# TorontoDeepLearning/convnet

Hardware: AMD Instinct MI355X
Metric: images/sec (fprop+bprop+wgrad) AlexNet 224x224 bs=256 (higher is better)
Workload: dtype f32

## Files before the change

convnet_amd/csrc/elementwise.hip:

```cpp
#include <cfloat>
#include <climits>
#include <cmath>

#include "common.h"

namespace chip {

using f32x4 = __attribute__((ext_vector_type(4))) float;

constexpr int kThreads = 256;
constexpr int kMaxBlocks = 2048;

inline int blocks_for(size_t work_items) {
  size_t b = (work_items + kThreads - 1) / kThreads;
  if (b > kMaxBlocks) b = kMaxBlocks;
  if (b < 1) b = 1;
  return (int)b;
}

template <typename F>
__global__ void map2_kernel(float* __restrict__ out, const float* a, const float* b, size_t n, bool vec, F f) {
  const size_t tid = (size_t)blockIdx.x * blockDim.x + threadIdx.x, stride = (size_t)gridDim.x * blockDim.x;
  if (vec) {
    const size_t n4 = n >> 2;
// ... 194 lines not shown
}

__global__ void add_row_kernel(float* __restrict__ out, const float* __restrict__ mat, const float* __restrict__ vec, int rows,
                               size_t n, float mult, bool vec4) {
  const size_t tid = (size_t)blockIdx.x * blockDim.x + threadIdx.x, stride = (size_t)gridDim.x * blockDim.x;
  if (vec4) {
    for (size_t i = tid; i < (n >> 2); i += stride) {
      const float b = mult * vec[(i << 2) / rows];
      f32x4 v = reinterpret_cast<const f32x4*>(mat)[i];
      v = v + b;
      reinterpret_cast<f32x4*>(out)[i] = v;
    }
  } else {
    for (size_t i = tid; i < n; i += stride) out[i] = mat[i] + mult * vec[i / rows];
  }
}

int add_row(cudamat* mat, cudamat* vec, cudamat* target, float mult) {
  if (!mat->on_device || !vec->on_device || !target->on_device) return ERROR_NOT_ON_DEVICE;
  if (mat->is_trans) return ERROR_TRANSPOSED;
  if (mat->size[1] != vec->size[1] || vec->size[0] != 1 || mat->size[0] != target->size[0] || mat->size[1] != target->size[1])
    return ERROR_INCOMPATIBLE_DIMENSIONS;
  const size_t n = numel(mat);
  const bool v4 = (mat->size[0] & 3) == 0 && aligned16(mat->data_device) && aligned16(target->data_device);
  hipLaunchKernelGGL(add_row_kernel, dim3(blocks_for(n / 4 + 1)), dim3(kThreads), 0, stream(), target->data_device, mat->data_device,
                     vec->data_device, mat->size[0], n, mult, v4);
  return launch_status();
}

__device__ __forceinline__ void sgd_one(float& g, float& w, float& h, float l2, float clip, float eps, float mom);

template <bool DO_SGD>
__global__ void rows_sq_kernel(float* __restrict__ g, float* __restrict__ w, float* __restrict__ h, int rows, int cols, int chunk,
                               float* __restrict__ partial, float l2, float clip, float eps, float mom) {
  const int r = blockIdx.x * blockDim.x + threadIdx.x;
  if (r >= rows) return;
  const int c0 = blockIdx.y * chunk, c1 = min(cols, c0 + chunk);
  float s = 0.f;
  for (int c = c0; c < c1; ++c) {
    const size_t i = (size_t)r + (size_t)rows * c;
    float wv = w[i];
    if (DO_SGD) {
      float gv = g[i], hv = h[i];
      sgd_one(gv, wv, hv, l2, clip, eps, mom);
      g[i] = gv;
      h[i] = hv;
      w[i] = wv;
    }
    s += wv * wv;
  }
  partial[(size_t)blockIdx.y * rows + r] = s;
}

template <bool DO_SGD>
__global__ void rows_sq4_kernel(float* __restrict__ g, float* __restrict__ w, float* __restrict__ h, int rows, int cols, int chunk,
                                float* __restrict__ partial, float l2, float clip, float eps, float mom) {
  const int r = 4 * (blockIdx.x * blockDim.x + threadIdx.x);
  if (r >= rows) return;
  const int c0 = blockIdx.y * chunk, c1 = min(cols, c0 + chunk);
  f32x4 s = {0.f, 0.f, 0.f, 0.f};
  auto one = [&](int c) {
    const size_t i = (size_t)r + (size_t)rows * c;
    f32x4 wv = *reinterpret_cast<f32x4*>(w + i);
    if (DO_SGD) {
      f32x4 gv = *reinterpret_cast<f32x4*>(g + i), hv = *reinterpret_cast<f32x4*>(h + i);
#pragma unroll
      for (int e = 0; e < 4; ++e) {
        float a = gv[e], b = wv[e], d = hv[e];
        sgd_one(a, b, d, l2, clip, eps, mom);
        gv[e] = a; wv[e] = b; hv[e] = d;
      }
      *reinterpret_cast<f32x4*>(g + i) = gv;
      *reinterpret_cast<f32x4*>(h + i) = hv;
      *reinterpret_cast<f32x4*>(w + i) = wv;
    }
    s += wv * wv;
  };
  int c = c0;
  for (; c + 1 < c1; c += 2) {
    one(c);
    one(c + 1);
  }
  if (c < c1) one(c);
  *reinterpret_cast<f32x4*>(partial + (size_t)blockIdx.y * rows + r) = s;
}

__global__ void row_factor_kernel(const float* __restrict__ partial, int nchunks, int rows, float norm, int constraint, float* __restrict__ factor) {
  __shared__ float sh[4][64];
  const int r = blockIdx.x * 64 + (threadIdx.x & 63), q = threadIdx.x >> 6;
  float s = 0.f;
  if (r < rows)
    for (int k = q; k < nchunks; k += 4) s += partial[(size_t)k * rows + r];
  sh[q][threadIdx.x & 63] = s;
  __syncthreads();
  if (q != 0 || r >= rows) return;
  s = sqrtf((sh[0][threadIdx.x] + sh[1][threadIdx.x]) + (sh[2][threadIdx.x] + sh[3][threadIdx.x]));
  factor[r] = (constraint == 1 || s > norm) ? norm / s : 1.f;
}

__global__ void row_scale_kernel(const float* __restrict__ src, float* __restrict__ dst, int rows, int cols, int chunk, const float* __restrict__ factor) {
  const int r = blockIdx.x * blockDim.x + threadIdx.x;
  const float f = r < rows ? factor[r] : 1.f;
  const bool in_place = src == dst;
  if (in_place && !__syncthreads_or(f != 1.f)) return;
  if (r >= rows) return;
  const int c0 = blockIdx.y * chunk, c1 = min(cols, c0 + chunk);
  for (int c = c0; c < c1; ++c) {
    const size_t i = (size_t)r + (size_t)rows * c;
    dst[i] = src[i] * f;
  }
}

inline int rows_normlimit(float* g, float* w_in, float* w_out, float* h, int rows, int cols, float norm, int constraint, bool do_sgd,
                          float l2, float clip, float eps, float mom) {
  int chunk = 64;
  while ((long)divup(rows, 256) * divup(cols, chunk) > 4096 && chunk < cols) chunk *= 2;
  const int nchunks = divup(cols, chunk);
  float* partial = static_cast<float*>(workspace(sizeof(float) * ((size_t)nchunks * rows + rows)));
  float* factor = partial + (size_t)nchunks * rows;
  dim3 grid(divup(rows, 256), nchunks);
  const bool v4 = (rows & 3) == 0 && aligned16(w_in) && (!do_sgd || (aligned16(g) && aligned16(h)));
  KernelTimer timer(do_sgd ? "rows_sq_kernel<sgd> + row_scale_kernel" : "rows_sq_kernel + row_scale_kernel", do_sgd ? "sgd_normlimit" : "normlimit", 0.0,
                    4.0 * (double)rows * cols * (do_sgd ? 7 : 3));
  if (v4) {
    const dim3 g4(divup(rows / 4, 64), nchunks);
    if (do_sgd)
      hipLaunchKernelGGL(rows_sq4_kernel<true>, g4, dim3(64), 0, stream(), g, w_in, h, rows, cols, chunk, partial, l2, clip, eps, mom);
    else
      hipLaunchKernelGGL(rows_sq4_kernel<false>, g4, dim3(64), 0, stream(), nullptr, w_in, nullptr, rows, cols, chunk, partial, 0.f, 0.f, 0.f, 0.f);
  } else if (do_sgd)
    hipLaunchKernelGGL(rows_sq_kernel<true>, grid, dim3(256), 0, stream(), g, w_in, h, rows, cols, chunk, partial, l2, clip, eps, mom);
  else
    hipLaunchKernelGGL(rows_sq_kernel<false>, grid, dim3(256), 0, stream(), nullptr, w_in, nullptr, rows, cols, chunk, partial, 0.f, 0.f, 0.f, 0.f);
  hipLaunchKernelGGL(row_factor_kernel, dim3(divup(rows, 64)), dim3(256), 0, stream(), partial, nchunks, rows, norm, constraint, factor);
  hipLaunchKernelGGL(row_scale_kernel, grid, dim3(256), 0, stream(), w_in, w_out, rows, cols, chunk, factor);
  return launch_status();
}

__global__ void normlimit_cols_kernel(const float* __restrict__ mat, float* __restrict__ target, int rows, float norm, int constraint) {
  __shared__ float sh[8];
  const float* col = mat + (size_t)blockIdx.x * rows;
  float* out = target + (size_t)blockIdx.x * rows;
  float s = 0.f;
  for (int i = threadIdx.x; i < rows; i += blockDim.x) s += col[i] * col[i];
  s = sqrtf(block_sum(s, sh));
  const float sc = (constraint == 1 || s > norm) ? norm / s : 1.f;
  for (int i = threadIdx.x; i < rows; i += blockDim.x) out[i] = col[i] * sc;
}

struct SoftmaxOut {
  float* probs;
  float* deriv;
  float* correct;
};

template <int G>
__global__ void __launch_bounds__(G * 32) softmax_rows_kernel(const float* logits, const float* __restrict__ labels, SoftmaxOut o, int rows, int cols, float deriv_scale) {
  __shared__ float red[G][33];
  __shared__ int redi[G][33];
  const int r = threadIdx.x & 31, g = threadIdx.x >> 5;
  const int row = blockIdx.x * 32 + r;
  const bool ok = row < rows;
  float mx = -FLT_MAX;
  int am = 0x7fffffff;
  if (ok)
    for (int j = g; j < cols; j += G) {
      const float v = logits[(size_t)j * rows + row];
      if (v > mx) { mx = v; am = j; }
    }
  red[g][r] = mx;
  redi[g][r] = am;
  __syncthreads();
  mx = red[0][r];
  am = redi[0][r];
#pragma unroll
  for (int k = 1; k < G; ++k) {
    const float v = red[k][r];
    const int a = redi[k][r];
    if (v > mx || (v == mx && a < am)) { mx = v; am = a; }
  }
  __syncthreads();
  float s = 0.f;
// ... 872 lines not shown
```

convnet_amd/csrc/gather_gemm.h:

```cpp
#pragma once
#include <cmath>
#include <cstring>
#include <type_traits>

#include "common.h"

namespace chip {

using f32x16 = __attribute__((ext_vector_type(16))) float;
using u32x4 = __attribute__((ext_vector_type(4))) unsigned;
using f32x4 = __attribute__((ext_vector_type(4))) float;

constexpr int BK = 16;

#ifdef CONVNET_GG_TRACE
constexpr bool kTrace = CONVNET_GG_TRACE >= 2;
__device__ unsigned long long* g_gg_trace = nullptr;
#else
constexpr bool kTrace = false;
#endif
__device__ __forceinline__ unsigned long long trace_clock() {
#ifdef CONVNET_GG_TRACE
  return __builtin_amdgcn_s_memtime();
#else
// ... 338 lines not shown

template <typename Acc>
__device__ __forceinline__ Acc split_mac(const Split8& a, const Split8& b, Acc v) {
  v = mma_bf16(a.m, b.m, v);
  v = mma_bf16(a.h, b.l, v);
  v = mma_bf16(a.l, b.h, v);
  v = mma_bf16(a.h, b.m, v);
  v = mma_bf16(a.m, b.h, v);
  v = mma_bf16(a.h, b.h, v);
  return v;
}

struct GGTile {
  const float* A;
  int K, GX, G, TX, TYX, y0, x0, dy0, dx0, ncols, col_tiles;
  int L, tsplit;
};
__device__ __forceinline__ bool gg_select_tile(const GGParams& p, const GGClassTable& ct, GGTile& t) {
  t.A = p.A; t.K = p.K; t.GX = p.GX; t.G = p.G; t.TX = p.TX; t.TYX = p.TYX; t.y0 = p.y0; t.x0 = p.x0; t.dy0 = p.dy0; t.dx0 = p.dx0;
  t.ncols = p.ncols; t.col_tiles = p.col_tiles; t.tsplit = -1;
  if (ct.n > 0) {
    const int b = blockIdx.x;
    if (b >= ct.c[ct.n - 1].tile_end) return false;
    int c = 0;
    while (b >= ct.c[c].tile_end) ++c;
    const int cbeg = c > 0 ? ct.c[c - 1].tile_end : 0;
    {
      const int i = b - cbeg, T = ct.c[c].tile_end - cbeg;
      const int q = T >> 3, m = T & 7, r = i & 7;
      t.L = r * q + (r < m ? r : m) + (i >> 3);
    }
    const GGClass& k = ct.c[c];
    t.A = k.A; t.K = k.K; t.GX = k.GX; t.G = k.G; t.TX = k.TX; t.TYX = k.TYX;
    t.y0 = k.y0; t.x0 = k.x0; t.dy0 = k.dy0; t.dx0 = k.dx0; t.ncols = k.ncols; t.col_tiles = k.col_tiles;
  } else if (p.tail_splits > 1) {
    const int k = blockIdx.x & 7, i = blockIdx.x >> 3;
    if (i < p.tail_tf8) {
      t.L = k * p.tail_tf8 + i;
    } else {
      const int j = k * p.tail_tt8 + (i - p.tail_tf8);
      if (j >= (p.row_tiles * t.col_tiles - p.tail_first) * p.tail_splits) return false;
      t.L = p.tail_first + j / p.tail_splits;
      t.tsplit = j % p.tail_splits;
    }
  } else {
    const int tiles = p.row_tiles * t.col_tiles;
    const int per = (tiles + 7) >> 3;
    t.L = xcd_remap(blockIdx.x, tiles);
    if (t.L >= tiles || (int)blockIdx.x >= per * 8) return false;
  }
  return true;
}

constexpr int kTailFixParts = 4;
template <int WR, int WC, int MT, int CW, bool VEC>
__global__ __launch_bounds__(WR* WC * 64) void gg_tail_fix_kernel(const GGParams p) {
  constexpr int NT = WR * WC * 64, NTC = CW / 32, ROWS = WR * MT * 32;
  using fvec = __attribute__((ext_vector_type(NTC))) float;
  const int tile = blockIdx.x / kTailFixParts, part = blockIdx.x % kTailFixParts;
  const int L = p.tail_first + tile;
  const int tid = threadIdx.x;
  const int reg_lo = part * (16 / kTailFixParts), reg_hi = reg_lo + 16 / kTailFixParts;
  f32x16 acc[MT][NTC];
  const float* pp = p.tail_partial + (size_t)tile * p.tail_splits * (size_t)(ROWS * WC * CW);
#pragma unroll
  for (int t = 0; t < MT; ++t)
#pragma unroll
    for (int reg = 0; reg < 16; ++reg) {
      if (reg < reg_lo || reg >= reg_hi) continue;
      fvec v = *reinterpret_cast<const fvec*>(pp + ((size_t)(t * 16 + reg) * NT + tid) * NTC);
      for (int sp = 1; sp < p.tail_splits; ++sp)
        v += *reinterpret_cast<const fvec*>(pp + (size_t)sp * (ROWS * WC * CW) + ((size_t)(t * 16 + reg) * NT + tid) * NTC);
#pragma unroll
      for (int u = 0; u < NTC; ++u) acc[t][u][reg] = v[u];
    }
  gg_epilogue<WR, WC, MT, CW, VEC>(p, acc, L % p.row_tiles, L / p.row_tiles, 0, p.ncols, p.GX, p.G, p.dy0, p.dx0, reg_lo, reg_hi);
}

struct PatchBank {
  const float* W;
  int F, C, Ky, Kx, cy, cx, sy, sx, TYc, TXc;
  bool dgrad;
};
void filter_planes_rt_launch(const PatchBank& bank, void* out, int TYX, int TH, const char* op);
void filter_planes_gk_launch(const float* W, void* out, int F, int K, int KP, int TH, const char* op);
bool patch_shape_ok(GGParams& p, size_t dst_elems);
void patch_run(GGParams& p, size_t dst_elems, const char* op, double flops, const PatchBank& bank);
bool patch_classes_ok(const GGParams& base, const GGClassTable& ct);
void patch_run_classes(GGParams& p, GGClassTable& ct, const char* op, double flops, double exec);

bool gfc_try(const float* images, const float* filters, const float* bias, float* targets, int N, int C, int H, int W, int F, int Ky, int Kx,
             int sy, int sx, int pady, int padx, int My, int Mx, float scaleTargets, int relu, double flops);

struct WGParams {
  const float* src;
  const float* dout;
  float* dst;
  float* partial;
  const float* zero;
  float* bias_dst;
  int K, F, N;
  int GX, M;
  int TX, TYX;
  int SH, SW;
  int ssy, ssx, y0, x0;
  int nchunk;
  int chunks_total;
  int chunks_per_split;
  int splits;
  int k_tiles, f_tiles;
  float scaleTargets, scaleOutput;
  int prio;
  int wide;
};

constexpr int WG_NB = 32;
constexpr int WG_PITCH = WG_NB + 4;

void wg_reduce_launch(const WGParams& p, size_t total, int splits, int groups, const char* op);
float* wg_batch_partial(const WGParams& p, size_t total, int splits);
bool wgw_try(WGParams& p, bool vec, bool split_products, const char* op, double flops, double exec);

void gg_reduce_launch(const GGParams& p, size_t dst_elems, int splits, const char* op);

inline double gg_split_time(int tiles, int sp, double slots, double tile_flops, double block_rate, size_t dst_elems) {
  const double rounds = std::ceil(tiles * (double)sp / slots);
  double t = rounds * (tile_flops / sp) / block_rate;
  if (sp > 1) t += sizeof(float) * (double)dst_elems * (2.0 * sp + 1) / 4.0e12 + 4e-6;
  return t;
// ... 44 lines not shown
```

convnet_amd/csrc/gather_gemm.hip:

```cpp
#include <algorithm>
#include <array>
#include <cmath>
#include <map>
#include <vector>
#include <cstdlib>
#include <string>
#include <type_traits>

#include "common.h"

#include "gather_gemm.h"

namespace chip {

template <int WR, int WC, int MT, int CW, bool A_KCONTIG, bool VEC, bool O3 = false, bool SPLIT = false>
__global__ __launch_bounds__(WR* WC * 64, (O3 ? 3 : 2)) void gg_kernel(const GGParams pin, const GGClassTable ct) {
  constexpr int NT = WR * WC * 64;
  constexpr int NTC = CW / 32, CW4 = CW / 4;
  using fvec = __attribute__((ext_vector_type(NTC))) float;
  constexpr int ROWS = WR * MT * 32;
  constexpr int APITCH = A_KCONTIG ? (BK + 4) : ROWS;
  constexpr int A_STAGE = A_KCONTIG ? ROWS * APITCH : BK * ROWS;
  constexpr int B_STAGE = WC * BK * CW;
  constexpr int NA = ((A_KCONTIG ? ROWS * (BK / 4) : BK * (ROWS / 4)) + NT - 1) / NT;
// ... 733 lines not shown
#pragma unroll
    for (int t = 0; t < MT; ++t) a[0][t] = ar[lh * ROWS + t * 32];
    b4[0] = *reinterpret_cast<const fvec*>(bs + lh * BROW);
    static_for<0, BK / 2>([&](auto KK) __attribute__((always_inline)) {
      constexpr int kk = decltype(KK)::value;
      constexpr int cur = kk & 1, nxt = cur ^ 1;
      if constexpr (kk + 1 < BK / 2) {
        const int krow = 2 * (kk + 1) + lh;
#pragma unroll
        for (int t = 0; t < MT; ++t) a[nxt][t] = ar[krow * ROWS + t * 32];
        b4[nxt] = *reinterpret_cast<const fvec*>(bs + krow * BROW);
      }
      __builtin_amdgcn_sched_barrier(0);
#pragma unroll
      for (int t = 0; t < MT; ++t)
#pragma unroll
        for (int u = 0; u < NTC; ++u)
          acc[t][u] = __builtin_amdgcn_mfma_f32_32x32x2f32(a[cur][t], b4[cur][u], acc[t][u], 0, 0, 0);
    });
    stage = stage == ST - 1 ? 0 : stage + 1;
    __syncthreads();
  }

  if (tsplit >= 0) {
    float* pp = p.tail_partial + ((size_t)(L - p.tail_first) * p.tail_splits + tsplit) * (size_t)(ROWS * WC * CW);
#pragma unroll
    for (int t = 0; t < MT; ++t)
#pragma unroll
      for (int reg = 0; reg < 16; ++reg) {
        fvec v;
#pragma unroll
        for (int u = 0; u < NTC; ++u) v[u] = acc[t][u][reg];
        *reinterpret_cast<fvec*>(pp + ((size_t)(t * 16 + reg) * NC + tid) * NTC) = v;
      }
    return;
  }
  gg_epilogue<WR, WC, MT, CW, true>(p, acc, row_tile, col_tile, split, T.ncols, T.GX, T.G, T.dy0, T.dx0);
}

__global__ void gg_reduce_kernel(float* __restrict__ dst, const float* __restrict__ partial, const float* __restrict__ bias,
                                 size_t total, size_t slab, int splits, size_t per_row, float scaleTargets, int relu,
                                 const float* __restrict__ mask, float post_scale) {
  for (size_t i = (size_t)blockIdx.x * blockDim.x + threadIdx.x; i < total; i += (size_t)gridDim.x * blockDim.x) {
    float s = 0.f;
    for (int k = 0; k < splits; ++k) s += partial[(size_t)k * slab + i];
    if (scaleTargets != 0.f) s = scaleTargets * dst[i] + s;
    if (bias) s += bias[i / per_row];
    if (relu) s = s > 0.f ? s : 0.f;
    if (mask) s = mask[i] > 0.f ? s * post_scale : 0.f;
    dst[i] = s;
  }
}

__global__ void dgrad_filter_kernel(const float* __restrict__ W, float* __restrict__ Wt, int F, int C, int Ky, int Kx, int cy,
                                    int cx, int sy, int sx, int TYc, int TXc, int tap_major) {
  const size_t total = (size_t)C * TXc * TYc * F;
  for (size_t i = (size_t)blockIdx.x * blockDim.x + threadIdx.x; i < total; i += (size_t)gridDim.x * blockDim.x) {
    const int c = i % C;
    size_t r = i / C;
    int a, b, f;
    if (tap_major) {
      const int f16 = r % 16;
      r /= 16;
      const int tap = r % (TXc * TYc);
      const int fb = r / (TXc * TYc);
      f = fb * 16 + f16;
      a = tap / TXc;
      b = tap - a * TXc;
    } else {
      b = r % TXc;
      r /= TXc;
      a = r % TYc;
      f = r / TYc;
    }
    Wt[i] = W[(size_t)f + (size_t)F * ((cx + sx * b) + Kx * ((cy + sy * a) + Ky * c))];
  }
}

__global__ void filter_tapmajor_kernel(const float* __restrict__ W, float* __restrict__ Wt, int F, int C, int TYX) {
  const size_t total = (size_t)F * C * TYX;
  for (size_t i = (size_t)blockIdx.x * blockDim.x + threadIdx.x; i < total; i += (size_t)gridDim.x * blockDim.x) {
    const int f = i % F;
    size_t r = i / F;
    const int c16 = r % 16;
    r /= 16;
    const int tap = r % TYX;
    const int c = (int)(r / TYX) * 16 + c16;
    Wt[i] = W[(size_t)f + (size_t)F * (tap + (size_t)TYX * c)];
  }
}

template <int WM, int WN, int MT, int NTL, bool VEC, int TS, bool SPLIT = false>
__global__ __launch_bounds__(WM* WN * 64) void wg_kernel(const WGParams p) {
  constexpr int NT = WM * WN * 64;
  constexpr int KT = WM * MT * TS;
  constexpr int FT = WN * NTL * TS;
  constexpr int LH = 64 / TS;
  using facc = __attribute__((ext_vector_type(TS == 32 ? 16 : 4))) float;
  constexpr int PITCH = VEC ? WG_NB : WG_PITCH;
  constexpr int A_STAGE = KT * PITCH, B_STAGE = FT * PITCH;
  constexpr int NA = (KT * 8 + NT - 1) / NT, NB = (FT * 8 + NT - 1) / NT;
  extern __shared__ __attribute__((aligned(16))) float smem[];
  float* As = smem;
  float* Bs = smem + 2 * A_STAGE;

  const int tiles = p.k_tiles * p.f_tiles;
// ... 250 lines not shown
        if (fin) {
          v = v * p.scaleOutput;
          if (p.scaleTargets != 0.f) v = p.scaleTargets * ld4(dp) + v;
        }
        st4(dp, v);
      }
      return;
    }
  }
#pragma unroll
  for (int u = 0; u < NTL; ++u) {
    const int f = f0 + (wn * NTL + u) * TS + li;
    if (f >= p.F) continue;
#pragma unroll
    for (int t = 0; t < MT; ++t) {
#pragma unroll
      for (int reg = 0; reg < (TS == 32 ? 16 : 4); ++reg) {
        const int k = kc0 + (wm * MT + t) * TS + (TS == 32 ? (reg & 3) + 8 * (reg >> 2) + 4 * lh : 4 * lh + reg);
        if (k >= KB) continue;
        float* dp = (fin && k == p.K) ? p.bias_dst + f : out + (size_t)k * p.F + f;
        float v = acc[t][u][reg];
        if (fin) {
          v *= p.scaleOutput;
          if (p.scaleTargets != 0.f) v = p.scaleTargets * (*dp) + v;
        }
        *dp = v;
      }
    }
  }
}

__global__ void wg_reduce_group_kernel(float* __restrict__ stage, const float* __restrict__ partial, size_t total, int splits, int per) {
  const int g = blockIdx.y;
  const int k0 = g * per, k1 = min(splits, k0 + per);
  for (size_t i = (size_t)blockIdx.x * blockDim.x + threadIdx.x; i < total; i += (size_t)gridDim.x * blockDim.x) {
    float s = 0.f;
    for (int k = k0; k < k1; ++k) s += partial[(size_t)k * total + i];
    stage[(size_t)g * total + i] = s;
  }
}

__global__ void wg_reduce_kernel(float* __restrict__ dst, float* __restrict__ dst2, const float* __restrict__ partial, size_t total,
                                 size_t main, int splits, float scaleTargets, float scaleOutput) {
  for (size_t i = (size_t)blockIdx.x * blockDim.x + threadIdx.x; i < total; i += (size_t)gridDim.x * blockDim.x) {
    float s = 0.f;
    for (int k = 0; k < splits; ++k) s += partial[(size_t)k * total + i];
    s *= scaleOutput;
    float* d = i < main ? dst + i : dst2 + (i - main);
    if (scaleTargets != 0.f) s = scaleTargets * (*d) + s;
    *d = s;
  }
}

__global__ void __launch_bounds__(256) dot_generic_kernel(const float* __restrict__ a, const float* __restrict__ b, float* __restrict__ c, int m, int n,
                                                          int k, int ld1, int ld2, int t1, int t2, float beta, float alpha) {
  __shared__ float As[32][33], Bs[32][33];
  const int tx = threadIdx.x & 31, ty = threadIdx.x >> 5;
  const int i0 = blockIdx.x * 32, j0 = blockIdx.y * 32;
  float acc[4] = {0.f, 0.f, 0.f, 0.f};
  for (int l0 = 0; l0 < k; l0 += 32) {
    for (int r = ty; r < 32; r += 8) {
      if (t1) {
        const int i = i0 + r, l = l0 + tx;
        As[tx][r] = (i < m && l < k) ? a[(size_t)l + (size_t)ld1 * i] : 0.f;
      } else {
        const int i = i0 + tx, l = l0 + r;
        As[r][tx] = (i < m && l < k) ? a[(size_t)i + (size_t)ld1 * l] : 0.f;
      }
      if (t2) {
        const int j = j0 + tx, l = l0 + r;
        Bs[r][tx] = (j < n && l < k) ? b[(size_t)j + (size_t)ld2 * l] : 0.f;
      } else {
        const int j = j0 + r, l = l0 + tx;
        Bs[tx][r] = (j < n && l < k) ? b[(size_t)l + (size_t)ld2 * j] : 0.f;
      }
    }
    __syncthreads();
#pragma unroll 8
    for (int l = 0; l < 32; ++l) {
      const float av = As[l][tx];
#pragma unroll
      for (int q = 0; q < 4; ++q) acc[q] = fmaf(av, Bs[l][ty + 8 * q], acc[q]);
    }
    __syncthreads();
  }
  const int i = i0 + tx;
  if (i < m) {
#pragma unroll
    for (int q = 0; q < 4; ++q) {
      const int j = j0 + ty + 8 * q;
      if (j < n) {
        float* d = c + (size_t)i + (size_t)m * j;
        *d = (beta != 0.f ? beta * (*d) : 0.f) + alpha * acc[q];
      }
    }
  }
}

namespace {

constexpr int kTargetBlocks = 512;

struct GGTimer {
  const char* op;
  double flops, exec;
};
// ... 155 lines not shown
  const int tiles = p.row_tiles * p.col_tiles;
  const int kchunks = divup(p.K, BK);
  const bool no_o3 = CHIP_DIAG_KNOB("CONVNET_GG_NO_O3", 0) != 0;
  const bool o3 = !no_o3 && !gg_split_mode() && vec && !AK && WR == 2 && WC == 2 && MT == 2 && CW == 128 && tiles >= 2 * 768 && p.KC == 0;
  int slots = o3 ? 768 : kTargetBlocks;
  if constexpr (kHasProducer<WC, CW, AK>) {
    if (p.KC > 0) slots = ggp_slots<WR, WC, MT, CW>(gg_split_mode(), p.apre != 0);
  }
  const double block_rate = gg_split_mode() ? 190e12 / slots : 64.0 * 4 * 2.2e9 * 0.8 / 2;
  const double flops = 2.0 * ROWS * (WC * (double)CW) * (double)p.K;
  const bool may_tail = dst_elems > 0 && gg_partial_last_round(tiles, slots, kchunks) && !CHIP_DIAG_KNOB("CONVNET_GG_NO_TAIL_SPLIT", 0);
  double best_t = 1e30;
  int splits = gg_split_k(tiles, slots, flops, block_rate, dst_elems, kchunks, kchunks, &best_t);
  int tail_s_instead = 0;
  if (splits > 1 && may_tail) {
    const int full = (tiles / slots) * slots, rem = tiles - full;
    const double t_round = flops / block_rate, tile_bytes = sizeof(float) * (double)ROWS * WC * CW;
    for (int s = 2; s <= 8 && kchunks / s >= 8; ++s) {
      const double t = (full / (double)slots + std::ceil(rem * (double)s / (double)slots) / s) * t_round + rem * (s + 1.0) * tile_bytes / 4.0e12 + 6e-6;
      if (t < best_t) {
        splits = 1;
        tail_s_instead = s;
        break;
      }
    }
  }
  p.chunks_per_split = kchunks > 0 ? divup(kchunks, splits) : 1;
  splits = kchunks > 0 ? divup(kchunks, p.chunks_per_split) : 1;
  p.splits = splits;
  p.slab = dst_elems;
  p.partial = splits > 1 ? static_cast<float*>(workspace(sizeof(float) * dst_elems * splits)) : nullptr;
  p.tail_splits = 1;
  p.tail_partial = nullptr;
  if (splits == 1 && may_tail) {
    int best_s = gg_tail_split(tiles, slots, flops, block_rate, TILE, kchunks);
    if (best_s == 1 && tail_s_instead > 1) best_s = tail_s_instead;
    if (best_s > 1) gg_set_tail(p, tiles, slots, kchunks, best_s, TILE);
  }
  dim3 grid(p.tail_splits > 1 ? 8 * (p.tail_tf8 + p.tail_tt8) : ((tiles + 7) / 8) * 8, splits);
  gg_launch_variant<WR, WC, MT, CW, AK>(p, kNoClasses, vec, o3, grid, lds_pad, tm);
  if (p.tail_splits > 1) {
    const int rem = tiles - p.tail_first;
    KernelTimer timer("gg_tail_fix_kernel", tm.op, 0.0, sizeof(float) * (double)rem * (p.tail_splits + 1) * ROWS * WC * CW);
    if (vec) hipLaunchKernelGGL((gg_tail_fix_kernel<WR, WC, MT, CW, true>), dim3(rem * kTailFixParts), dim3(WR * WC * 64), 0, stream(), p);
    else hipLaunchKernelGGL((gg_tail_fix_kernel<WR, WC, MT, CW, false>), dim3(rem * kTailFixParts), dim3(WR * WC * 64), 0, stream(), p);
  }
  if (splits > 1) gg_reduce_launch(p, dst_elems, splits, tm.op);
}

}

void wg_reduce_launch(const WGParams& p, size_t total, int splits, int groups, const char* op) {
  KernelTimer timer("wg_reduce_kernel", op, 0.0, sizeof(float) * (double)total * (splits + 1));
  size_t nb = (total + 255) / 256;
  if (nb > 4096) nb = 4096;
  const float* slabs = p.partial;
  int nslabs = splits;
  if (groups > 1) {
    float* stage = p.partial + (size_t)splits * total;
    const int per = divup(splits, groups);
    hipLaunchKernelGGL(wg_reduce_group_kernel, dim3((unsigned)nb, divup(splits, per)), dim3(256), 0, stream(), stage, p.partial, total, splits, per);
    slabs = stage;
    nslabs = divup(splits, per);
  }
  hipLaunchKernelGGL(wg_reduce_kernel, dim3((unsigned)nb), dim3(256), 0, stream(), p.dst, p.bias_dst, slabs, total, (size_t)p.K * p.F, nslabs,
                     p.scaleTargets, p.scaleOutput);
}

namespace {
struct WGBatch {
  int frames = 0, frame = 0, splits = 0;
  size_t total = 0;
  void* (*arena)(size_t) = nullptr;
  size_t max_bytes = 0;
  WGParams last;
};
WGBatch g_wgb;
}
void wg_batch_begin(int frames, void* (*slab_arena)(size_t), size_t max_bytes) {
  g_wgb = WGBatch{};
  g_wgb.frames = frames;
  g_wgb.arena = slab_arena;
  g_wgb.max_bytes = max_bytes;
}
bool wg_batch_active() { return g_wgb.frames > 0; }
int wg_batch_frame() { return g_wgb.frame; }
float* wg_batch_partial(const WGParams& p, size_t total, int splits) {
  WGBatch& b = g_wgb;
  if (!b.frames) return nullptr;
  CHIP_REQUIRE(b.frame < b.frames);
  const size_t S = (size_t)b.frames * splits;
  const size_t bytes = sizeof(float) * total * (S + (S > 64 ? 32 : 0));
  if (b.frame == 0) {
    if (bytes > b.max_bytes) {
      b.frames = 0;
      return nullptr;
    }
    b.splits = splits;
    b.total = total;
  }
  CHIP_REQUIRE(b.splits == splits && b.total == total);
  float* arena = static_cast<float*>(b.arena(bytes));
  b.last = p;
  b.last.partial = arena;
  return arena + (size_t)b.frame++ * splits * total;
}
void wg_batch_end() {
  WGBatch& b = g_wgb;
  if (b.frames && b.frame > 0) {
    CHIP_REQUIRE(b.frame == b.frames);
    const int S = b.frames * b.splits;
    wg_reduce_launch(b.last, b.total, S, S > 64 ? 32 : 1, "conv_wgrad");
  }
  b.frames = 0;
}

void gg_reduce_launch(const GGParams& p, size_t dst_elems, int splits, const char* op) {
  KernelTimer timer("gg_reduce_kernel", op, 0.0, sizeof(float) * (double)dst_elems * (splits + 1));
  size_t nb = (dst_elems + 255) / 256;
  if (nb > 4096) nb = 4096;
  hipLaunchKernelGGL(gg_reduce_kernel, dim3((unsigned)nb), dim3(256), 0, stream(), p.dst, p.partial, p.bias, dst_elems, p.slab, splits,
                     (size_t)p.DP * p.N, p.scaleTargets, p.relu, p.mask, p.post_scale);
}

namespace {

template <bool AK>
void gg_run(GGParams& p, bool vec, size_t dst_elems, const GGTimer& tm) {
  gg_with_tile(gg_tile(p.R, vec, p.skinny != 0), [&](auto t) {
    using T = decltype(t);
    gg_launch_cfg<T::WR, T::WC, T::MT, T::CW, AK>(p, vec, dst_elems, tm);
  });
}

void gg_run_classes(GGParams& p, GGClassTable& ct, bool vec, const GGTimer& tm) {
  gg_with_tile(gg_tile(p.R, vec, false), [&](auto t) {
    using T = decltype(t);
    gg_launch_classes<T::WR, T::WC, T::MT, T::CW>(p, ct, vec, tm);
  });
}

template <int WM, int WN, int MT, int NTL, int TS = 32>
void wg_launch_cfg(WGParams& p, bool vec, const GGTimer& tm) {
  constexpr int KT = WM * MT * TS, FT = WN * NTL * TS;
  const size_t lds = sizeof(float) * 2 * (KT + FT) * (vec ? WG_NB : WG_PITCH);
  p.k_tiles = divup(p.K, KT);
  if (p.bias_dst && divup(p.K + 1, KT) != p.k_tiles) p.bias_dst = nullptr;
  p.f_tiles = divup(p.F, FT);
  p.zero = zero_page();
  p.prio = wg_prio_mode();
  const int tiles = p.k_tiles * p.f_tiles;
  const size_t total = (size_t)(p.K + (p.bias_dst ? 1 : 0)) * p.F;
  const bool no_wide = CHIP_DIAG_KNOB("CONVNET_WG_NO_WIDE", 0) != 0;
  p.wide = (!no_wide && vec && TS == 32 && WM == 2 && WN == 2 && MT == 2 && NTL == 2 && p.F % 4 == 0 && aligned16(p.dst) &&
            (!p.bias_dst || aligned16(p.bias_dst))) ? 1 : 0;
  int splits = 1;
  if (tiles < kTargetBlocks) {
    splits = kTargetBlocks / tiles;
    const int max_by_len = p.chunks_total / 16 > 0 ? p.chunks_total / 16 : 1;
    if (splits > max_by_len) splits = max_by_len;
    const size_t max_by_bytes = (size_t(256) << 20) / (total * sizeof(float)) + 1;
    if ((size_t)splits > max_by_bytes) splits = (int)max_by_bytes;
    if (splits > 1024) splits = 1024;
    if (splits < 1) splits = 1;
  }
  p.chunks_per_split = divup(p.chunks_total, splits);
  splits = divup(p.chunks_total, p.chunks_per_split);
  p.splits = splits;
  const int groups = splits > 64 ? 32 : 1;
  float* const frame_slabs = wg_batch_partial(p, total, splits);
  p.partial = frame_slabs ? frame_slabs
                          : splits > 1 ? static_cast<float*>(workspace(sizeof(float) * total * (splits + (groups > 1 ? groups : 0)))) : nullptr;
  dim3 grid(((tiles * splits + 7) / 8) * 8), block(WM * WN * 64);
  static const std::string kname_f = "wg_kernel<" + std::to_string(WM) + "," + std::to_string(WN) + "," + std::to_string(MT) + "," + std::to_string(NTL) + (TS == 16 ? ",x16>" : ">");
  static const std::string kname_s = kname_f.substr(0, kname_f.size() - 1) + ",split>";
// ... 451 lines not shown
```

convnet_amd/csrc/patch_gemm.hip:

```cpp
#include <algorithm>
#include <cmath>
#include <cstdlib>
#include <string>

#include "gather_gemm.h"

#ifndef CONVNET_GPV_LDS_MAP
#define CONVNET_GPV_LDS_MAP 0
#endif
#ifndef CONVNET_GPV_FILT_LATE
#define CONVNET_GPV_FILT_LATE 1
#endif

namespace chip {

__global__ void __launch_bounds__(256) act_planes_kernel(const float* __restrict__ src, u32x4* __restrict__ out, int CB, int HW, int N4) {
  const size_t total = (size_t)CB * 2 * HW * N4;
  const size_t cstride = (size_t)HW * N4 * 4;
  const int IB = N4 / 16;
  for (size_t i = (size_t)blockIdx.x * blockDim.x + threadIdx.x; i < total; i += (size_t)gridDim.x * blockDim.x) {
    const int n4 = (int)(i % N4);
    size_t r = i / N4;
    const int pix = (int)(r % HW);
    r /= HW;
// ... 914 lines not shown
        split_pair(0, 2, fn);
        mac_step(K4{}, fa, fc, NTC - 1);
        split_pair(0, 3, fn);
        mac_step(K5{}, fa, fc, NTC - 1);
        CHIP_PIN_SPLIT8(fn);
        __builtin_amdgcn_sched_barrier(0);
      }
    };
    load_a(0, fa0);
    read_b();
#pragma unroll
    for (int q = 0; q < 4; ++q) split_pair(0, q, fb[0]);
    int c = 0;
    if (nchunks & 1) {
      chunk(fa0, fa1);
      c = 1;
    } else {
#pragma unroll
      for (int t = 0; t < MT; ++t) fa1[t] = fa0[t];
    }
    for (; c < nchunks; c += 2) {
      chunk(fa1, fa0);
      chunk(fa0, fa1);
    }
    __builtin_amdgcn_s_waitcnt(0x0070);
  }

  acc_settle();
  if (tsplit >= 0) {
    float* pp = p.tail_partial + ((size_t)(L - p.tail_first) * p.tail_splits + tsplit) * (size_t)(ROWS * WC * CW);
#pragma unroll
    for (int t = 0; t < MT; ++t)
#pragma unroll
      for (int reg = 0; reg < 16; ++reg) {
        fvec v;
#pragma unroll
        for (int u = 0; u < NTC; ++u) v[u] = acc_elem<true>(acc[t][u][reg]);
        *reinterpret_cast<fvec*>(pp + ((size_t)(t * 16 + reg) * NC + tid) * NTC) = v;
      }
    return;
  }
  gg_epilogue<1, WC, MT, CW, true, true>(p, acc, row_tile, col_tile, split, T.ncols, T.GX, T.G, T.dy0, T.dx0);
}

template <int MT, int PART>
__device__ __forceinline__ void gpw_tail_fix_part(const GGParams& p, int tile) {
  constexpr int WC = 4, CW = 128, NT = WC * 64, NTC = CW / 32, ROWS = MT * 32;
  constexpr int reg_lo = PART * (16 / kTailFixParts), reg_hi = reg_lo + 16 / kTailFixParts;
  using fvec = __attribute__((ext_vector_type(NTC))) float;
  const int L = p.tail_first + tile;
  const int tid = threadIdx.x;
  f32x16 acc[MT][NTC];
  const float* pp = p.tail_partial + (size_t)tile * p.tail_splits * (size_t)(ROWS * WC * CW);
#pragma unroll
  for (int t = 0; t < MT; ++t)
#pragma unroll
    for (int reg = reg_lo; reg < reg_hi; ++reg) {
      fvec v = *reinterpret_cast<const fvec*>(pp + ((size_t)(t * 16 + reg) * NT + tid) * NTC);
      for (int sp = 1; sp < p.tail_splits; ++sp)
        v += *reinterpret_cast<const fvec*>(pp + (size_t)sp * (ROWS * WC * CW) + ((size_t)(t * 16 + reg) * NT + tid) * NTC);
#pragma unroll
      for (int u = 0; u < NTC; ++u) acc[t][u][reg] = v[u];
    }
  gg_epilogue<1, WC, MT, CW, true>(p, acc, L % p.row_tiles, L / p.row_tiles, 0, p.ncols, p.GX, p.G, p.dy0, p.dx0, reg_lo, reg_hi);
}
template <int MT>
__global__ __launch_bounds__(256) void gpw_tail_fix_kernel(const GGParams p) {
  const int tile = blockIdx.x / kTailFixParts;
  switch (blockIdx.x % kTailFixParts) {
    case 0: gpw_tail_fix_part<MT, 0>(p, tile); break;
    case 1: gpw_tail_fix_part<MT, 1>(p, tile); break;
    case 2: gpw_tail_fix_part<MT, 2>(p, tile); break;
    default: gpw_tail_fix_part<MT, 3>(p, tile); break;
  }
}

template <int MT>
__global__ __launch_bounds__(256, 1) void gpv_kernel(const GGParams pin, const GGClassTable ct) {
  constexpr int WC = 4, CW = 128, NTC = CW / 32, P = kWideP, NS = kWideNS;
  using fvec = __attribute__((ext_vector_type(NTC))) float;
  constexpr int NC = WC * 64;
  constexpr int ROWS = MT * 32;
  constexpr int A_STAGE = 6 * ROWS * 4;
  constexpr int STA = 3;
  constexpr int SLAB = NS * 1024;
  constexpr unsigned A_WAVE = A_STAGE * 4 / WC;
  static_assert(MT == 4 || MT == 3, "a wave's share of a filter chunk is three pieces, or two and a quarter");
  extern __shared__ __attribute__((aligned(16))) float smem[];
#if CONVNET_GPV_LDS_MAP == 1
  constexpr int A_STRIDE = A_STAGE + SLAB, B_STRIDE = A_STAGE + SLAB;
  float* As = smem;
  float* Bs = smem + A_STAGE;
  float* const dump_slot = smem + STA * A_STAGE + 2 * SLAB;
#else
  constexpr int A_STRIDE = A_STAGE, B_STRIDE = SLAB;
  float* As = smem;
  float* Bs = smem + STA * A_STAGE;
  float* const dump_slot = smem + STA * A_STAGE + 2 * SLAB;
#endif

  const GGParams& p = pin;
  GGTile T;
  if (!gg_select_tile(p, ct, T)) return;
  const int L = T.L, tsplit = T.tsplit;
  const int row_tile = L % p.row_tiles, col_tile = L / p.row_tiles;
  const int split = blockIdx.y;
  const int tid = threadIdx.x;
  const int wave = __builtin_amdgcn_readfirstlane(tid >> 6), lane = tid & 63;
  const int li = lane & 31, lh = lane >> 5;
  const int N = p.N;
  const int dir = p.dir, SH = p.SH, SW = p.SW, ssx = p.ssx;
  auto sgpr = [](int v) __attribute__((always_inline)) { return __builtin_amdgcn_readfirstlane(v); };

  const int TX = sgpr(T.TX), TYX = sgpr(T.TYX), TYn = sgpr(TYX / TX);
  const int ng = ssx;
  const int cnt0 = sgpr(ssx == 1 ? TX : (TX + 1) >> 1), cnt1 = sgpr(ssx == 1 ? TX : TX >> 1);
  const int gb00 = sgpr(dir > 0 ? 0 : (cnt0 - 1) * ssx), gb01 = sgpr(ssx == 1 ? gb00 : dir > 0 ? 1 : 1 + (cnt1 - 1) * ssx);
  const int dstep = dir * ssx;

  const int G = T.G, GX = T.GX, units = p.IB * G;
  int ys_f = 1 << 30, ys_l = -(1 << 30);
  int S_l = 0, my_ord[3] = {-1, -1, -1};
  int sy_l = 0, sx_l = 0, sib_l = 0, imin_l = 3;
  {
    int S[P], oy[P], ox[P], ib[P];
    bool ok[P];
// ... 687 lines not shown
```

Before: 27580.

## Vectorize and batch loads in split-K reductions, tail-fix and norm-limit kernels

```diff
diff --git a/convnet_amd/csrc/elementwise.hip b/convnet_amd/csrc/elementwise.hip
--- a/convnet_amd/csrc/elementwise.hip
+++ b/convnet_amd/csrc/elementwise.hip
@@ -270,18 +270,17 @@
   partial[(size_t)blockIdx.y * rows + r] = s;
 }
 
+constexpr int kRowsSqCols = 8;
+constexpr int kRowsSqBlock = 128;
 template <bool DO_SGD>
-__global__ void rows_sq4_kernel(float* __restrict__ g, float* __restrict__ w, float* __restrict__ h, int rows, int cols, int chunk,
-                                float* __restrict__ partial, float l2, float clip, float eps, float mom) {
+__global__ __launch_bounds__(kRowsSqBlock) void rows_sq4_kernel(float* __restrict__ g, float* __restrict__ w, float* __restrict__ h, int rows, int cols,
+                                                       int chunk, float* __restrict__ partial, float l2, float clip, float eps, float mom) {
   const int r = 4 * (blockIdx.x * blockDim.x + threadIdx.x);
   if (r >= rows) return;
   const int c0 = blockIdx.y * chunk, c1 = min(cols, c0 + chunk);
   f32x4 s = {0.f, 0.f, 0.f, 0.f};
-  auto one = [&](int c) {
-    const size_t i = (size_t)r + (size_t)rows * c;
-    f32x4 wv = *reinterpret_cast<f32x4*>(w + i);
+  auto one = [&](size_t i, f32x4 gv, f32x4 wv, f32x4 hv) {
     if (DO_SGD) {
-      f32x4 gv = *reinterpret_cast<f32x4*>(g + i), hv = *reinterpret_cast<f32x4*>(h + i);
 #pragma unroll
       for (int e = 0; e < 4; ++e) {
         float a = gv[e], b = wv[e], d = hv[e];
@@ -295,11 +294,29 @@
     s += wv * wv;
   };
   int c = c0;
-  for (; c + 1 < c1; c += 2) {
-    one(c);
-    one(c + 1);
-  }
-  if (c < c1) one(c);
+  for (; c + kRowsSqCols <= c1; c += kRowsSqCols) {
+    f32x4 gv[kRowsSqCols], wv[kRowsSqCols], hv[kRowsSqCols];
+#pragma unroll
+    for (int u = 0; u < kRowsSqCols; ++u) {
+      const size_t i = (size_t)r + (size_t)rows * (c + u);
+      wv[u] = *reinterpret_cast<const f32x4*>(w + i);
+      if (DO_SGD) {
+        gv[u] = *reinterpret_cast<const f32x4*>(g + i);
+        hv[u] = *reinterpret_cast<const f32x4*>(h + i);
+      }
+    }
+#pragma unroll
+    for (int u = 0; u < kRowsSqCols; ++u) one((size_t)r + (size_t)rows * (c + u), gv[u], wv[u], hv[u]);
+  }
+  for (; c < c1; ++c) {
+    const size_t i = (size_t)r + (size_t)rows * c;
+    f32x4 gv, hv, wv = *reinterpret_cast<const f32x4*>(w + i);
+    if (DO_SGD) {
+      gv = *reinterpret_cast<const f32x4*>(g + i);
+      hv = *reinterpret_cast<const f32x4*>(h + i);
+    }
+    one(i, gv, wv, hv);
+  }
   *reinterpret_cast<f32x4*>(partial + (size_t)blockIdx.y * rows + r) = s;
 }
 
@@ -308,7 +325,14 @@
   const int r = blockIdx.x * 64 + (threadIdx.x & 63), q = threadIdx.x >> 6;
   float s = 0.f;
   if (r < rows)
-    for (int k = q; k < nchunks; k += 4) s += partial[(size_t)k * rows + r];
+    for (int k = q; k < nchunks; k += 4 * 8) {
+      float v[8];
+#pragma unroll
+      for (int u = 0; u < 8; ++u) v[u] = k + 4 * u < nchunks ? partial[(size_t)(k + 4 * u) * rows + r] : 0.f;
+#pragma unroll
+      for (int u = 0; u < 8; ++u)
+        if (k + 4 * u < nchunks) s += v[u];
+    }
   sh[q][threadIdx.x & 63] = s;
   __syncthreads();
   if (q != 0 || r >= rows) return;
@@ -341,11 +365,11 @@
   KernelTimer timer(do_sgd ? "rows_sq_kernel<sgd> + row_scale_kernel" : "rows_sq_kernel + row_scale_kernel", do_sgd ? "sgd_normlimit" : "normlimit", 0.0,
                     4.0 * (double)rows * cols * (do_sgd ? 7 : 3));
   if (v4) {
-    const dim3 g4(divup(rows / 4, 64), nchunks);
+    const dim3 g4(divup(rows / 4, kRowsSqBlock), nchunks);
     if (do_sgd)
-      hipLaunchKernelGGL(rows_sq4_kernel<true>, g4, dim3(64), 0, stream(), g, w_in, h, rows, cols, chunk, partial, l2, clip, eps, mom);
+      hipLaunchKernelGGL(rows_sq4_kernel<true>, g4, dim3(kRowsSqBlock), 0, stream(), g, w_in, h, rows, cols, chunk, partial, l2, clip, eps, mom);
     else
-      hipLaunchKernelGGL(rows_sq4_kernel<false>, g4, dim3(64), 0, stream(), nullptr, w_in, nullptr, rows, cols, chunk, partial, 0.f, 0.f, 0.f, 0.f);
+      hipLaunchKernelGGL(rows_sq4_kernel<false>, g4, dim3(kRowsSqBlock), 0, stream(), nullptr, w_in, nullptr, rows, cols, chunk, partial, 0.f, 0.f, 0.f, 0.f);
   } else if (do_sgd)
     hipLaunchKernelGGL(rows_sq_kernel<true>, grid, dim3(256), 0, stream(), g, w_in, h, rows, cols, chunk, partial, l2, clip, eps, mom);
   else
diff --git a/convnet_amd/csrc/gather_gemm.h b/convnet_amd/csrc/gather_gemm.h
--- a/convnet_amd/csrc/gather_gemm.h
+++ b/convnet_amd/csrc/gather_gemm.h
@@ -414,29 +414,55 @@
   return true;
 }
 
-constexpr int kTailFixParts = 4;
+constexpr int kTailFixParts = 8;
+template <int WR, int WC, int MT, int CW, bool VEC, int PART>
+__device__ __forceinline__ void gg_tail_fix_part(const GGParams& p, int tile) {
+  constexpr int NT = WR * WC * 64, NTC = CW / 32, ROWS = WR * MT * 32, PR = 16 / kTailFixParts;
+  constexpr int reg_lo = PART * PR, reg_hi = reg_lo + PR;
+  using fvec = __attribute__((ext_vector_type(NTC))) float;
+  const int L = p.tail_first + tile;
+  const int tid = threadIdx.x;
+  f32x16 acc[MT][NTC];
+  const float* pp = p.tail_partial + (size_t)tile * p.tail_splits * (size_t)(ROWS * WC * CW);
+  fvec v[MT][PR];
+#pragma unroll
+  for (int t = 0; t < MT; ++t)
+#pragma unroll
+    for (int j = 0; j < PR; ++j) v[t][j] = *reinterpret_cast<const fvec*>(pp + ((size_t)(t * 16 + reg_lo + j) * NT + tid) * NTC);
+  for (int sp = 1; sp < p.tail_splits; ++sp) {
+    fvec x[MT][PR];
+#pragma unroll
+    for (int t = 0; t < MT; ++t)
+#pragma unroll
+      for (int j = 0; j < PR; ++j)
+        x[t][j] = *reinterpret_cast<const fvec*>(pp + (size_t)sp * (ROWS * WC * CW) + ((size_t)(t * 16 + reg_lo + j) * NT + tid) * NTC);
+#pragma unroll
+    for (int t = 0; t < MT; ++t)
+#pragma unroll
+      for (int j = 0; j < PR; ++j) v[t][j] += x[t][j];
+  }
+#pragma unroll
+  for (int t = 0; t < MT; ++t)
+#pragma unroll
+    for (int j = 0; j < PR; ++j)
+#pragma unroll
+      for (int u = 0; u < NTC; ++u) acc[t][u][reg_lo + j] = v[t][j][u];
+  gg_epilogue<WR, WC, MT, CW, VEC>(p, acc, L % p.row_tiles, L / p.row_tiles, 0, p.ncols, p.GX, p.G, p.dy0, p.dx0, reg_lo, reg_hi);
+}
 template <int WR, int WC, int MT, int CW, bool VEC>
 __global__ __launch_bounds__(WR* WC * 64) void gg_tail_fix_kernel(const GGParams p) {
-  constexpr int NT = WR * WC * 64, NTC = CW / 32, ROWS = WR * MT * 32;
-  using fvec = __attribute__((ext_vector_type(NTC))) float;
-  const int tile = blockIdx.x / kTailFixParts, part = blockIdx.x % kTailFixParts;
-  const int L = p.tail_first + tile;
-  const int tid = threadIdx.x;
-  const int reg_lo = part * (16 / kTailFixParts), reg_hi = reg_lo + 16 / kTailFixParts;
-  f32x16 acc[MT][NTC];
-  const float* pp = p.tail_partial + (size_t)tile * p.tail_splits * (size_t)(ROWS * WC * CW);
-#pragma unroll
-  for (int t = 0; t < MT; ++t)
-#pragma unroll
-    for (int reg = 0; reg < 16; ++reg) {
-      if (reg < reg_lo || reg >= reg_hi) continue;
-      fvec v = *reinterpret_cast<const fvec*>(pp + ((size_t)(t * 16 + reg) * NT + tid) * NTC);
-      for (int sp = 1; sp < p.tail_splits; ++sp)
-        v += *reinterpret_cast<const fvec*>(pp + (size_t)sp * (ROWS * WC * CW) + ((size_t)(t * 16 + reg) * NT + tid) * NTC);
-#pragma unroll
-      for (int u = 0; u < NTC; ++u) acc[t][u][reg] = v[u];
-    }
-  gg_epilogue<WR, WC, MT, CW, VEC>(p, acc, L % p.row_tiles, L / p.row_tiles, 0, p.ncols, p.GX, p.G, p.dy0, p.dx0, reg_lo, reg_hi);
+  static_assert(kTailFixParts == 8, "one case per part");
+  const int tile = blockIdx.x / kTailFixParts;
+  switch (blockIdx.x % kTailFixParts) {
+    case 0: gg_tail_fix_part<WR, WC, MT, CW, VEC, 0>(p, tile); break;
+    case 1: gg_tail_fix_part<WR, WC, MT, CW, VEC, 1>(p, tile); break;
+    case 2: gg_tail_fix_part<WR, WC, MT, CW, VEC, 2>(p, tile); break;
+    case 3: gg_tail_fix_part<WR, WC, MT, CW, VEC, 3>(p, tile); break;
+    case 4: gg_tail_fix_part<WR, WC, MT, CW, VEC, 4>(p, tile); break;
+    case 5: gg_tail_fix_part<WR, WC, MT, CW, VEC, 5>(p, tile); break;
+    case 6: gg_tail_fix_part<WR, WC, MT, CW, VEC, 6>(p, tile); break;
+    default: gg_tail_fix_part<WR, WC, MT, CW, VEC, 7>(p, tile); break;
+  }
 }
 
 struct PatchBank {
diff --git a/convnet_amd/csrc/gather_gemm.hip b/convnet_amd/csrc/gather_gemm.hip
--- a/convnet_amd/csrc/gather_gemm.hip
+++ b/convnet_amd/csrc/gather_gemm.hip
@@ -809,6 +809,50 @@
   }
 }
 
+constexpr int kSlabLoads = 8;
+__device__ __forceinline__ f32x4 slab_sum4(const float* __restrict__ partial, size_t stride, size_t i, int k0, int k1) {
+  f32x4 s = {0.f, 0.f, 0.f, 0.f};
+  int k = k0;
+  for (; k + kSlabLoads <= k1; k += kSlabLoads) {
+    f32x4 v[kSlabLoads];
+#pragma unroll
+    for (int u = 0; u < kSlabLoads; ++u) v[u] = *reinterpret_cast<const f32x4*>(partial + (size_t)(k + u) * stride + i);
+#pragma unroll
+    for (int u = 0; u < kSlabLoads; ++u) s += v[u];
+  }
+  if (k + 4 <= k1) {
+    f32x4 v[4];
+#pragma unroll
+    for (int u = 0; u < 4; ++u) v[u] = *reinterpret_cast<const f32x4*>(partial + (size_t)(k + u) * stride + i);
+#pragma unroll
+    for (int u = 0; u < 4; ++u) s += v[u];
+    k += 4;
+  }
+  for (; k < k1; ++k) s += *reinterpret_cast<const f32x4*>(partial + (size_t)k * stride + i);
+  return s;
+}
+
+template <bool DIV64>
+__global__ __launch_bounds__(256) void gg_reduce4_kernel(float* __restrict__ dst, const float* __restrict__ partial, const float* __restrict__ bias,
+                                                         size_t total, size_t slab, int splits, size_t per_row, float scaleTargets, int relu,
+                                                         const float* __restrict__ mask, float post_scale) {
+  for (size_t i = 4 * ((size_t)blockIdx.x * blockDim.x + threadIdx.x); i < total; i += 4 * (size_t)gridDim.x * blockDim.x) {
+    f32x4 s = slab_sum4(partial, slab, i, 0, splits);
+    if (scaleTargets != 0.f) s = scaleTargets * *reinterpret_cast<const f32x4*>(dst + i) + s;
+    if (bias) s += bias[DIV64 ? i / per_row : (size_t)((unsigned)i / (unsigned)per_row)];
+    if (relu) {
+#pragma unroll
+      for (int e = 0; e < 4; ++e) s[e] = s[e] > 0.f ? s[e] : 0.f;
+    }
+    if (mask) {
+      const f32x4 mk = *reinterpret_cast<const f32x4*>(mask + i);
+#pragma unroll
+      for (int e = 0; e < 4; ++e) s[e] = mk[e] > 0.f ? s[e] * post_scale : 0.f;
+    }
+    *reinterpret_cast<f32x4*>(dst + i) = s;
+  }
+}
+
 __global__ void dgrad_filter_kernel(const float* __restrict__ W, float* __restrict__ Wt, int F, int C, int Ky, int Kx, int cy,
                                     int cx, int sy, int sx, int TYc, int TXc, int tap_major) {
   const size_t total = (size_t)C * TXc * TYc * F;
@@ -1165,6 +1209,24 @@
   }
 }
 
+__global__ __launch_bounds__(256) void wg_reduce_group4_kernel(float* __restrict__ stage, const float* __restrict__ partial, size_t total,
+                                                               int splits, int per) {
+  const int g = blockIdx.y;
+  const int k0 = g * per, k1 = min(splits, k0 + per);
+  for (size_t i = 4 * ((size_t)blockIdx.x * blockDim.x + threadIdx.x); i < total; i += 4 * (size_t)gridDim.x * blockDim.x)
+    *reinterpret_cast<f32x4*>(stage + (size_t)g * total + i) = slab_sum4(partial, total, i, k0, k1);
+}
+__global__ __launch_bounds__(256) void wg_reduce4_kernel(float* __restrict__ dst, float* __restrict__ dst2, const float* __restrict__ partial,
+                                                         size_t total, size_t main, int splits, float scaleTargets, float scaleOutput) {
+  for (size_t i = 4 * ((size_t)blockIdx.x * blockDim.x + threadIdx.x); i < total; i += 4 * (size_t)gridDim.x * blockDim.x) {
+    f32x4 s = slab_sum4(partial, total, i, 0, splits);
+    s *= scaleOutput;
+    f32x4* d = reinterpret_cast<f32x4*>(i < main ? dst + i : dst2 + (i - main));
+    if (scaleTargets != 0.f) s = scaleTargets * (*d) + s;
+    *d = s;
+  }
+}
+
 __global__ void __launch_bounds__(256) dot_generic_kernel(const float* __restrict__ a, const float* __restrict__ b, float* __restrict__ c, int m, int n,
                                                           int k, int ld1, int ld2, int t1, int t2, float beta, float alpha) {
   __shared__ float As[32][33], Bs[32][33];
@@ -1426,19 +1488,28 @@
 
 void wg_reduce_launch(const WGParams& p, size_t total, int splits, int groups, const char* op) {
   KernelTimer timer("wg_reduce_kernel", op, 0.0, sizeof(float) * (double)total * (splits + 1));
-  size_t nb = (total + 255) / 256;
+  const size_t main = (size_t)p.K * p.F;
+  const bool v4 = total % 4 == 0 && main % 4 == 0 && aligned16(p.partial) && aligned16(p.dst) && (main == total || aligned16(p.bias_dst));
+  size_t nb = ((v4 ? total / 4 : total) + 255) / 256;
   if (nb > 4096) nb = 4096;
   const float* slabs = p.partial;
   int nslabs = splits;
   if (groups > 1) {
     float* stage = p.partial + (size_t)splits * total;
     const int per = divup(splits, groups);
-    hipLaunchKernelGGL(wg_reduce_group_kernel, dim3((unsigned)nb, divup(splits, per)), dim3(256), 0, stream(), stage, p.partial, total, splits, per);
+    if (v4)
+      hipLaunchKernelGGL(wg_reduce_group4_kernel, dim3((unsigned)nb, divup(splits, per)), dim3(256), 0, stream(), stage, p.partial, total, splits, per);
+    else
+      hipLaunchKernelGGL(wg_reduce_group_kernel, dim3((unsigned)nb, divup(splits, per)), dim3(256), 0, stream(), stage, p.partial, total, splits, per);
     slabs = stage;
     nslabs = divup(splits, per);
   }
-  hipLaunchKernelGGL(wg_reduce_kernel, dim3((unsigned)nb), dim3(256), 0, stream(), p.dst, p.bias_dst, slabs, total, (size_t)p.K * p.F, nslabs,
-                     p.scaleTargets, p.scaleOutput);
+  if (v4)
+    hipLaunchKernelGGL(wg_reduce4_kernel, dim3((unsigned)nb), dim3(256), 0, stream(), p.dst, p.bias_dst, slabs, total, main, nslabs, p.scaleTargets,
+                       p.scaleOutput);
+  else
+    hipLaunchKernelGGL(wg_reduce_kernel, dim3((unsigned)nb), dim3(256), 0, stream(), p.dst, p.bias_dst, slabs, total, main, nslabs, p.scaleTargets,
+                       p.scaleOutput);
 }
 
 namespace {
@@ -1491,10 +1562,19 @@
 
 void gg_reduce_launch(const GGParams& p, size_t dst_elems, int splits, const char* op) {
   KernelTimer timer("gg_reduce_kernel", op, 0.0, sizeof(float) * (double)dst_elems * (splits + 1));
-  size_t nb = (dst_elems + 255) / 256;
+  const size_t per_row = (size_t)p.DP * p.N;
+  const bool v4 = dst_elems % 4 == 0 && p.slab % 4 == 0 && per_row % 4 == 0 && aligned16(p.dst) && aligned16(p.partial) && aligned16(p.mask);
+  size_t nb = ((v4 ? dst_elems / 4 : dst_elems) + 255) / 256;
   if (nb > 4096) nb = 4096;
-  hipLaunchKernelGGL(gg_reduce_kernel, dim3((unsigned)nb), dim3(256), 0, stream(), p.dst, p.partial, p.bias, dst_elems, p.slab, splits,
-                     (size_t)p.DP * p.N, p.scaleTargets, p.relu, p.mask, p.post_scale);
+  if (v4 && dst_elems < ((size_t)1 << 32))
+    hipLaunchKernelGGL(gg_reduce4_kernel<false>, dim3((unsigned)nb), dim3(256), 0, stream(), p.dst, p.partial, p.bias, dst_elems, p.slab, splits, per_row,
+                       p.scaleTargets, p.relu, p.mask, p.post_scale);
+  else if (v4)
+    hipLaunchKernelGGL(gg_reduce4_kernel<true>, dim3((unsigned)nb), dim3(256), 0, stream(), p.dst, p.partial, p.bias, dst_elems, p.slab, splits, per_row,
+                       p.scaleTargets, p.relu, p.mask, p.post_scale);
+  else
+    hipLaunchKernelGGL(gg_reduce_kernel, dim3((unsigned)nb), dim3(256), 0, stream(), p.dst, p.partial, p.bias, dst_elems, p.slab, splits, per_row,
+                       p.scaleTargets, p.relu, p.mask, p.post_scale);
 }
 
 namespace {
diff --git a/convnet_amd/csrc/patch_gemm.hip b/convnet_amd/csrc/patch_gemm.hip
--- a/convnet_amd/csrc/patch_gemm.hip
+++ b/convnet_amd/csrc/patch_gemm.hip
@@ -990,26 +990,44 @@
   const int tid = threadIdx.x;
   f32x16 acc[MT][NTC];
   const float* pp = p.tail_partial + (size_t)tile * p.tail_splits * (size_t)(ROWS * WC * CW);
+  fvec v[MT][reg_hi - reg_lo];
 #pragma unroll
   for (int t = 0; t < MT; ++t)
 #pragma unroll
-    for (int reg = reg_lo; reg < reg_hi; ++reg) {
-      fvec v = *reinterpret_cast<const fvec*>(pp + ((size_t)(t * 16 + reg) * NT + tid) * NTC);
-      for (int sp = 1; sp < p.tail_splits; ++sp)
-        v += *reinterpret_cast<const fvec*>(pp + (size_t)sp * (ROWS * WC * CW) + ((size_t)(t * 16 + reg) * NT + tid) * NTC);
-#pragma unroll
-      for (int u = 0; u < NTC; ++u) acc[t][u][reg] = v[u];
-    }
+    for (int reg = reg_lo; reg < reg_hi; ++reg) v[t][reg - reg_lo] = *reinterpret_cast<const fvec*>(pp + ((size_t)(t * 16 + reg) * NT + tid) * NTC);
+  for (int sp = 1; sp < p.tail_splits; ++sp) {
+    fvec x[MT][reg_hi - reg_lo];
+#pragma unroll
+    for (int t = 0; t < MT; ++t)
+#pragma unroll
+      for (int reg = reg_lo; reg < reg_hi; ++reg)
+        x[t][reg - reg_lo] = *reinterpret_cast<const fvec*>(pp + (size_t)sp * (ROWS * WC * CW) + ((size_t)(t * 16 + reg) * NT + tid) * NTC);
+#pragma unroll
+    for (int t = 0; t < MT; ++t)
+#pragma unroll
+      for (int reg = reg_lo; reg < reg_hi; ++reg) v[t][reg - reg_lo] += x[t][reg - reg_lo];
+  }
+#pragma unroll
+  for (int t = 0; t < MT; ++t)
+#pragma unroll
+    for (int reg = reg_lo; reg < reg_hi; ++reg)
+#pragma unroll
+      for (int u = 0; u < NTC; ++u) acc[t][u][reg] = v[t][reg - reg_lo][u];
   gg_epilogue<1, WC, MT, CW, true>(p, acc, L % p.row_tiles, L / p.row_tiles, 0, p.ncols, p.GX, p.G, p.dy0, p.dx0, reg_lo, reg_hi);
 }
 template <int MT>
 __global__ __launch_bounds__(256) void gpw_tail_fix_kernel(const GGParams p) {
+  static_assert(kTailFixParts == 8, "one case per part");
   const int tile = blockIdx.x / kTailFixParts;
   switch (blockIdx.x % kTailFixParts) {
     case 0: gpw_tail_fix_part<MT, 0>(p, tile); break;
     case 1: gpw_tail_fix_part<MT, 1>(p, tile); break;
     case 2: gpw_tail_fix_part<MT, 2>(p, tile); break;
-    default: gpw_tail_fix_part<MT, 3>(p, tile); break;
+    case 3: gpw_tail_fix_part<MT, 3>(p, tile); break;
+    case 4: gpw_tail_fix_part<MT, 4>(p, tile); break;
+    case 5: gpw_tail_fix_part<MT, 5>(p, tile); break;
+    case 6: gpw_tail_fix_part<MT, 6>(p, tile); break;
+    default: gpw_tail_fix_part<MT, 7>(p, tile); break;
   }
 }
 
```

Result: no change. 27680, median of 4 (+0.4%).
